# thuml/iVideoGPT

Measured on AMD Instinct MI355X. Metric: predicted frames/sec (encode+GPT rollout+decode), 64x64x16f, higher is better.
Workload: dtype bf16; 1 GPU; ivideogpt-oxe-64-act-free (BASELINE config 2): synthetic 64x64 bf16 clips, 64 trajectories per GPU, 2 context + 14 predicted frames, top-k 100 sampling, seeded random weights; global_batch=64, frames=16, resolution=64, lanes=4

## Files before the change

ivideogpt_amd/csrc/llama_ops.hip:

```cpp
#include <algorithm>
#include <cstdio>
#include <cstdlib>

#include "ops.h"
#include <atomic>
#include "switches.h"

namespace ivg {

template <typename T>
__global__ __launch_bounds__(256) void embed_kernel(const int64_t* __restrict__ ids, long id_stride, const T* __restrict__ E,
                                                    T* __restrict__ x, long x_bstride, int L, int H, int V) {
  constexpr int VEC = Traits<T>::VEC;
  const int row = blockIdx.x;
  const int b = row / L, l = row - b * L;
  long id = ids[(long)b * id_stride + l];
  id = id < 0 ? 0 : (id >= V ? V - 1 : id);
  const T* src = E + id * H;
  T* dst = x + (long)b * x_bstride + (long)l * H;
  for (int c = threadIdx.x * VEC; c < H; c += 256 * VEC) *(Chunk16*)(dst + c) = *(const Chunk16*)(src + c);
}

int launch_embed(const int64_t* ids, long id_stride, const void* E, void* x, DType dt, int B, int L, int H, int V, hipStream_t st,
                 long x_bstride) {
// ... 365 lines not shown
        }
        vf[d][pr] = bf16x8{half[0][0], half[0][1], half[0][2], half[0][3], half[1][0], half[1][1], half[1][2], half[1][3]};
      }
#pragma unroll
    for (int n = 0; n < NQ; ++n) {
      f32x4 sc[4];
      float mt = -INFINITY;
#pragma unroll
      for (int sub = 0; sub < 4; ++sub) {
        sc[sub] = f32x4{0.f, 0.f, 0.f, 0.f};
        sc[sub] = __builtin_amdgcn_mfma_f32_16x16x32_bf16(kf[sub][0], qf[n][0], sc[sub], 0, 0, 0);
        sc[sub] = __builtin_amdgcn_mfma_f32_16x16x32_bf16(kf[sub][1], qf[n][1], sc[sub], 0, 0, 0);
#pragma unroll
        for (int r = 0; r < 4; ++r) {
          const int key = k0 + sub * 16 + lg * 4 + r;
          sc[sub][r] = key <= qpos[n] ? sc[sub][r] * scale : -INFINITY;
          mt = fmaxf(mt, sc[sub][r]);
        }
      }
      mt = fmaxf(mt, __shfl_xor(mt, 16, 64));
      mt = fmaxf(mt, __shfl_xor(mt, 32, 64));
      const float mn = fmaxf(m[n], mt);
      const float ms = mn == -INFINITY ? 0.f : mn;
      const float alpha = expf(m[n] - ms);
      m[n] = mn;
      float ps = 0.f;
      bf16x8 pf[2];
#pragma unroll
      for (int sub = 0; sub < 4; ++sub)
#pragma unroll
        for (int r = 0; r < 4; ++r) {
          const float pw = expf(sc[sub][r] - ms);
          ps += pw;
          pf[sub >> 1][(sub & 1) * 4 + r] = (bf16_t)pw;
        }
      lsum[n] = lsum[n] * alpha + ps;
#pragma unroll
      for (int d = 0; d < 4; ++d) {
#pragma unroll
        for (int r = 0; r < 4; ++r) o[n][d][r] *= alpha;
#pragma unroll
        for (int pr = 0; pr < 2; ++pr) o[n][d] = __builtin_amdgcn_mfma_f32_16x16x32_bf16(vf[d][pr], pf[pr], o[n][d], 0, 0, 0);
      }
    }
  }
#pragma unroll
  for (int n = 0; n < NQ; ++n) {
    lsum[n] += __shfl_xor(lsum[n], 16, 64);
    lsum[n] += __shfl_xor(lsum[n], 32, 64);
    if (lg == 0) { sM[wave][n * 16 + lr] = m[n]; sL[wave][n * 16 + lr] = lsum[n]; }
  }
  __syncthreads();
  float* sO = (float*)sbuf;
  if (wave > 0) {
#pragma unroll
    for (int n = 0; n < NQ; ++n)
#pragma unroll
      for (int d = 0; d < 4; ++d)
#pragma unroll
        for (int r = 0; r < 4; ++r) sO[((((wave - 1) * NQ + n) * 4 + d) * 4 + r) * 64 + lane] = o[n][d][r];
  }
  __syncthreads();
  if (wave != 0) return;
#pragma unroll
  for (int n = 0; n < NQ; ++n) {
    const int qi = n * 16 + lr, t = t0 + qi;
    float M = m[n];
#pragma unroll
    for (int w = 1; w < 4; ++w) M = fmaxf(M, sM[w][qi]);
    const float s0 = expf(m[n] - M);
    float L = lsum[n] * s0;
    f32x4 acc[4];
#pragma unroll
    for (int d = 0; d < 4; ++d)
#pragma unroll
      for (int r = 0; r < 4; ++r) acc[d][r] = o[n][d][r] * s0;
#pragma unroll
    for (int w = 1; w < 4; ++w) {
      const float sw_ = expf(sM[w][qi] - M);
      L += sL[w][qi] * sw_;
#pragma unroll
      for (int d = 0; d < 4; ++d)
#pragma unroll
        for (int r = 0; r < 4; ++r) acc[d][r] += sO[((((w - 1) * NQ + n) * 4 + d) * 4 + r) * 64 + lane] * sw_;
    }
    if (t < T) {
      const float inv = 1.0f / L;
      bf16_t* orow = out + ((long)b * T + t) * H + h * HD + lg * 4;
#pragma unroll
      for (int d = 0; d < 4; ++d)
        *(bf16x4*)(orow + d * 16) = bf16x4{(bf16_t)(acc[d][0] * inv), (bf16_t)(acc[d][1] * inv), (bf16_t)(acc[d][2] * inv), (bf16_t)(acc[d][3] * inv)};
    }
  }
}

int launch_chunk_attn(const void* qkv, const void* kc, const void* vc, void* out, int B, int T, int heads, int hd, int Lmax, int pos0,
                      DType dt, hipStream_t st) {
  if (dt != BF16 || hd != 64 || B <= 0 || heads <= 0 || T < 1 || pos0 < 0 || (long)pos0 + T > Lmax) return -1;
  if (((uintptr_t)qkv & 15) || ((uintptr_t)out & 7) || ((uintptr_t)kc & 15) || ((uintptr_t)vc & 15)) return -1;
  const float scale = 1.0f / sqrtf((float)hd);
  if (T > 16)
    hipLaunchKernelGGL(chunk_attn_kernel<2>, dim3((unsigned)cdiv(T, 32), (unsigned)(B * heads)), dim3(256), 0, st, (const bf16_t*)qkv,
                       (const bf16_t*)kc, (const bf16_t*)vc, (bf16_t*)out, T, pos0, heads, Lmax, scale);
  else
    hipLaunchKernelGGL(chunk_attn_kernel<1>, dim3(1u, (unsigned)(B * heads)), dim3(256), 0, st, (const bf16_t*)qkv, (const bf16_t*)kc,
                       (const bf16_t*)vc, (bf16_t*)out, T, pos0, heads, Lmax, scale);
  return (int)hipGetLastError();
}

static std::atomic<long long> g_kv_extend_rows[2] = {{0}, {0}};
void kv_extend_note(int chunk_rows, int step_rows) { g_kv_extend_rows[0] += chunk_rows; g_kv_extend_rows[1] += step_rows; }
long long kv_extend_rows(int stepwise) { return g_kv_extend_rows[stepwise ? 1 : 0].load(); }
static std::atomic<long long> g_kv_extend_heads[2] = {{0}, {0}};
void kv_extend_heads_note(int frame_rows, int scored_rows) { g_kv_extend_heads[0] += frame_rows; g_kv_extend_heads[1] += scored_rows; }
long long kv_extend_heads_rows(int scored) { return g_kv_extend_heads[scored ? 1 : 0].load(); }

template <int HD, int KT, bool PRE = true>
__global__ __launch_bounds__(256) void xattn_kernel(const bf16_t* __restrict__ q, const bf16_t* __restrict__ Kp, const bf16_t* __restrict__ VpT,
                                                    bf16_t* __restrict__ out, int P, int kv, int C, int F, int nh, float scale) {
  constexpr int KQ = HD / 32;
  constexpr int DO = HD / 16;
  constexpr int SUB = KT / 16;
  constexpr int NPF = KT / 32;
  const int tid = threadIdx.x, wave = tid >> 6, lane = tid & 63, lr = lane & 15, lg = lane >> 4;
  const int qt = blockIdx.x;
  const int mh = blockIdx.y, m = mh / nh, h = mh - m * nh, b = m / F;
  const int qi = qt * 64 + wave * 16 + lr;
  const bf16_t* qrow = q + ((long)m * P + qi) * C + h * HD;
  bf16x8 qf[KQ];
#pragma unroll
  for (int k = 0; k < KQ; ++k) qf[k] = *(const bf16x8*)(qrow + k * 32 + lg * 8);
  const bf16_t* kb = Kp + (long)b * kv * C + h * HD;
  const bf16_t* vb = VpT + ((long)b * C + h * HD) * kv;
  f32x4 o[DO];
#pragma unroll
  for (int d = 0; d < DO; ++d) o[d] = f32x4{0.f, 0.f, 0.f, 0.f};
  float mx = -INFINITY, lsum = 0.f;
  constexpr int PK = HD + 16;
  using VT = VtTile<KT>;
  __shared__ __attribute__((aligned(16))) bf16_t sK[KT * PK];
  __shared__ __attribute__((aligned(16))) bf16_t sV[HD * VT::PITCH];
  constexpr int KC = KT * HD / 8 / 256;
  constexpr int VC = HD * KT / 8 / 256;
  constexpr int VCH = KT / 8;
  static_assert(KC >= 1 && VC >= 1, "tile too small for 256 threads");
  Chunk16 pk[KC], pvv[VC];
  auto fetch = [&](int kt) {
    const int k0 = kt * KT;
#pragma unroll
    for (int i = 0; i < KC; ++i) {
      const int c = i * 256 + tid, row = c / (HD / 8), col = (c % (HD / 8)) * 8;
      pk[i] = *(const Chunk16*)(kb + (long)(k0 + row) * C + col);
    }
#pragma unroll
    for (int i = 0; i < VC; ++i) {
      const int c = i * 256 + tid, row = c / VCH, col = (c % VCH) * 8;
      pvv[i] = *(const Chunk16*)(vb + (long)row * kv + k0 + col);
    }
  };
  const int ntiles = kv / KT;
  if constexpr (PRE) fetch(0);
  for (int kt = 0; kt < ntiles; ++kt) {
    __syncthreads();
    if constexpr (!PRE) fetch(kt);
#pragma unroll
    for (int i = 0; i < KC; ++i) { const int c = i * 256 + tid; *(Chunk16*)(sK + (c / (HD / 8)) * PK + (c % (HD / 8)) * 8) = pk[i]; }
#pragma unroll
    for (int i = 0; i < VC; ++i) { const int c = i * 256 + tid; VT::store(sV, c / VCH, c % VCH, pvv[i]); }
    __syncthreads();
    if constexpr (PRE) { if (kt + 1 < ntiles) fetch(kt + 1); }
    f32x4 sc[SUB];
    float mt = -INFINITY;
#pragma unroll
    for (int sub = 0; sub < SUB; ++sub) {
      sc[sub] = f32x4{0.f, 0.f, 0.f, 0.f};
      const bf16_t* krow = sK + (sub * 16 + lr) * PK + lg * 8;
#pragma unroll
      for (int k = 0; k < KQ; ++k) sc[sub] = __builtin_amdgcn_mfma_f32_16x16x32_bf16(*(const bf16x8*)(krow + k * 32), qf[k], sc[sub], 0, 0, 0);
#pragma unroll
      for (int r = 0; r < 4; ++r) { sc[sub][r] *= scale; mt = fmaxf(mt, sc[sub][r]); }
    }
    mt = fmaxf(mt, __shfl_xor(mt, 16, 64));
    mt = fmaxf(mt, __shfl_xor(mt, 32, 64));
    const float mn = fmaxf(mx, mt);
    const float alpha = expf(mx - mn);
    mx = mn;
    float ps = 0.f;
    bf16x8 pf[NPF];
#pragma unroll
    for (int sub = 0; sub < SUB; ++sub)
#pragma unroll
      for (int r = 0; r < 4; ++r) {
        const float pe = expf(sc[sub][r] - mn);
        ps += pe;
        pf[sub >> 1][(sub & 1) * 4 + r] = (bf16_t)pe;
      }
    lsum = lsum * alpha + ps;
#pragma unroll
    for (int d = 0; d < DO; ++d) {
#pragma unroll
      for (int r = 0; r < 4; ++r) o[d][r] *= alpha;
#pragma unroll
      for (int pr = 0; pr < NPF; ++pr)
        o[d] = __builtin_amdgcn_mfma_f32_16x16x32_bf16(VT::frag(sV, d * 16 + lr, pr * 4 + lg), pf[pr], o[d], 0, 0, 0);
    }
  }
  lsum += __shfl_xor(lsum, 16, 64);
  lsum += __shfl_xor(lsum, 32, 64);
  const float inv = 1.0f / lsum;
  bf16_t* orow = out + ((long)m * P + qi) * C + h * HD + lg * 4;
#pragma unroll
  for (int d = 0; d < DO; ++d)
    *(bf16x4*)(orow + d * 16) = bf16x4{(bf16_t)(o[d][0] * inv), (bf16_t)(o[d][1] * inv), (bf16_t)(o[d][2] * inv), (bf16_t)(o[d][3] * inv)};
}

bool xattn_covers(int P, int kv, int C, int nh, DType dt) {
  if (!sw().flash_xatt || dt != BF16 || nh <= 0 || C % nh != 0 || P % 64 != 0 || kv % 64 != 0 || (C & 7)) return false;
  const int hd = C / nh;
  return hd == 32 || hd == 64 || hd == 128 || hd == 192 || hd == 512 || hd == 768;
}

int launch_xattn(const void* q, const void* Kp, const void* VpT, void* out, int M, int F, int P, int kv, int C, int nh, DType dt, hipStream_t st) {
  if (!xattn_covers(P, kv, C, nh, dt) || M <= 0 || F <= 0 || M % F != 0) return -1;
  if (((uintptr_t)q & 15) || ((uintptr_t)Kp & 15) || ((uintptr_t)VpT & 15) || ((uintptr_t)out & 7)) return -1;
  const int hd = C / nh;
  dim3 grid((unsigned)(P / 64), (unsigned)(M * nh));
  const float scale = 1.0f / sqrtf((float)hd);
#define IVG_XATTN(HDv, KTv, PREv) hipLaunchKernelGGL((xattn_kernel<HDv, KTv, PREv>), grid, dim3(256), 0, st, (const bf16_t*)q, (const bf16_t*)Kp, (const bf16_t*)VpT, (bf16_t*)out, P, kv, C, F, nh, scale)
  if (hd == 128) IVG_XATTN(128, 64, true);
  else if (hd == 192) IVG_XATTN(192, 64, true);
  else if (hd == 64) IVG_XATTN(64, 64, true);
  else if (hd == 32) IVG_XATTN(32, 64, true);
  else if (hd == 512) IVG_XATTN(512, 32, true);
  else if (hd == 768) IVG_XATTN(768, 32, false);
  else return -1;
#undef IVG_XATTN
  return (int)hipGetLastError();
}

template <typename T> struct QPack;
template <> struct QPack<float> {
  __device__ __forceinline__ void set(const float*) {}
  __device__ __forceinline__ float dot(const float* qf, Chunk16 raw) const {
    const f32x4 kk = __builtin_bit_cast(f32x4, raw);
    float d = 0.f;
#pragma unroll
    for (int j = 0; j < 4; ++j) d = fmaf(qf[j], kk[j], d);
    return d;
  }
};
template <> struct QPack<bf16_t> {
  bf16x2 q[4];
  __device__ __forceinline__ void set(const float* qf) {
#pragma unroll
    for (int j = 0; j < 4; ++j) q[j] = bf16x2{(bf16_t)qf[2 * j], (bf16_t)qf[2 * j + 1]};
  }
  __device__ __forceinline__ float dot(const float*, Chunk16 raw) const {
    const bf16x8 kk = __builtin_bit_cast(bf16x8, raw);
    float d = 0.f;
#pragma unroll
    for (int j = 0; j < 4; ++j) d = __builtin_amdgcn_fdot2_f32_bf16(q[j], bf16x2{kk[2 * j], kk[2 * j + 1]}, d, false);
    return d;
  }
};
template <typename T> __device__ __forceinline__ float dot_chunk(const float* qf, Chunk16 raw) {
  constexpr int VEC = Traits<T>::VEC;
  float d = 0.f;
  if constexpr (sizeof(T) == 2) {
    const bf16x8 kk = __builtin_bit_cast(bf16x8, raw);
#pragma unroll
    for (int j = 0; j < VEC; ++j) d = fmaf(qf[j], (float)kk[j], d);
  } else {
    const f32x4 kk = __builtin_bit_cast(f32x4, raw);
#pragma unroll
    for (int j = 0; j < VEC; ++j) d = fmaf(qf[j], kk[j], d);
  }
  return d;
}
template <typename T> __device__ __forceinline__ void axpy_chunk(float* of, float pw, Chunk16 raw) {
  constexpr int VEC = Traits<T>::VEC;
  if constexpr (sizeof(T) == 2) {
    const bf16x8 vv = __builtin_bit_cast(bf16x8, raw);
#pragma unroll
    for (int j = 0; j < VEC; ++j) of[j] = fmaf(pw, (float)vv[j], of[j]);
  } else {
    const f32x4 vv = __builtin_bit_cast(f32x4, raw);
#pragma unroll
    for (int j = 0; j < VEC; ++j) of[j] = fmaf(pw, vv[j], of[j]);
  }
}

template <int CTRL> __device__ __forceinline__ float dpp_add(float v) {
  return v + __int_as_float(__builtin_amdgcn_update_dpp(0, __float_as_int(v), CTRL, 0xf, 0xf, false));
}
__device__ __forceinline__ float group_sum(float d, int lpk) {
  if (lpk >= 2) d = dpp_add<0xB1>(d);
  if (lpk >= 4) d = dpp_add<0x4E>(d);
  if (lpk >= 8) d = dpp_add<0x141>(d);
  if (lpk >= 16) d = dpp_add<0x140>(d);
  for (int o = 16; o < lpk; o <<= 1) d += __shfl_xor(d, o, 64);
  return d;
}

template <typename T, bool NT, int HD, bool SHARED = false>
__global__ __launch_bounds__(256) void decode_attn_kernel(const T* __restrict__ qkv, T* __restrict__ kc, T* __restrict__ vc,
                                                          T* __restrict__ out, const float* __restrict__ cosT,
                                                          const float* __restrict__ sinT, int heads, int hd_arg, int Lmax,
                                                          const StepState* __restrict__ state, unsigned long long* prof,
                                                          int sh_P = 0, int sh_G = 1, int sh_row0 = 0) {
  constexpr int VEC = Traits<T>::VEC;
  const int hd = HD > 0 ? HD : hd_arg;
  constexpr int UNR = 8;
  const unsigned long long t_start = prof ? wall_clock64() : 0ull;
  extern __shared__ __attribute__((aligned(16))) unsigned char smem[];
  const int lpk = hd / VEC;
  const int gpb = 256 / lpk;
  float* sq = (float*)smem;
  float* sk = sq + hd;
  float* sv = sk + hd;
  float* sc = sv + hd;
  float* red = sc + Lmax;
  __shared__ float sred[8];
  const int b = blockIdx.x / heads, h = blockIdx.x % heads;
  const int tid = threadIdx.x, lane = tid & 63, wv = tid >> 6;
  const int sub = tid % lpk, grp = tid / lpk;
  const int H = heads * hd, half = hd / 2;
  const float scale = rsqrtf((float)hd);
  T* kb = kc + ((long)b * heads + h) * Lmax * hd;
  T* vb = vc + ((long)b * heads + h) * Lmax * hd;
  long sh_delta = 0;
  if constexpr (SHARED) sh_delta = ((long)((b - sh_row0) / sh_G) - b) * heads * Lmax * hd * (long)sizeof(T);
  const int step = gpb * UNR;
  const unsigned lane_off = (unsigned)(sub * VEC) * (unsigned)sizeof(T);
  auto load_rows = [&](Chunk16 (&dst)[UNR], const T* base, int t0, int limit) {
    const char* bb = (const char*)base;
#pragma unroll
    for (int u = 0; u < UNR; ++u) {
      const int t = t0 + u * gpb + grp;
      const char* rb = bb;
      if constexpr (SHARED) rb = t < sh_P ? bb + sh_delta : bb;
      const Chunk16* src = (const Chunk16*)(rb + ((unsigned)(t * hd) * (unsigned)sizeof(T) + lane_off));
      dst[u] = t < limit ? ((NT && !SHARED) ? __builtin_nontemporal_load(src) : *src) : Chunk16{0u, 0u, 0u, 0u};
    }
  };
  Chunk16 cur[UNR], nxt[UNR];
  float rc = 0.f, rs = 0.f, q1 = 0.f, q2 = 0.f, k1 = 0.f, k2 = 0.f;
  T va = from_f32<T>(0.f), vb2 = from_f32<T>(0.f);
  if (tid < half) {
    const T* row = qkv + (long)b * 3 * H + h * hd;
    q1 = to_f32(row[tid]); q2 = to_f32(row[tid + half]);
    k1 = to_f32(row[H + tid]); k2 = to_f32(row[H + tid + half]);
    va = row[2 * H + tid]; vb2 = row[2 * H + tid + half];
  }
  load_rows(cur, kb, 0, Lmax);
  const int pos = state->pos;
  const int n_keys = pos + 1;
  if (tid < half) { rc = cosT[(long)pos * half + tid]; rs = sinT[(long)pos * half + tid]; }
  if (tid < half) {
    const T qa = from_f32<T>(q1 * rc - q2 * rs), qb = from_f32<T>(q2 * rc + q1 * rs);
    const T ka = from_f32<T>(k1 * rc - k2 * rs), kb2 = from_f32<T>(k2 * rc + k1 * rs);
    sq[tid] = to_f32(qa); sq[tid + half] = to_f32(qb);
    sk[tid] = to_f32(ka); sk[tid + half] = to_f32(kb2);
    sv[tid] = to_f32(va); sv[tid + half] = to_f32(vb2);
    kb[(long)pos * hd + tid] = ka; kb[(long)pos * hd + tid + half] = kb2;
    vb[(long)pos * hd + tid] = va; vb[(long)pos * hd + tid + half] = vb2;
  }
  __syncthreads();
  float qf[VEC];
#pragma unroll
  for (int j = 0; j < VEC; ++j) qf[j] = sq[sub * VEC + j];
  QPack<T> qp;
  qp.set(qf);
  auto scores = [&](Chunk16 (&rows)[UNR], int t0) {
#pragma unroll
    for (int u = 0; u < UNR; ++u) {
      const int t = t0 + u * gpb + grp;
      float d = qp.dot(qf, rows[u]);
      d = group_sum(d, lpk);
      if (t < pos && sub == 0) sc[t] = d * scale;
    }
  };
  {
    int t0 = 0;
    bool in_nxt = false;
    while (t0 < pos) {
      if (t0 + step < pos) load_rows(nxt, kb, t0 + step, pos); else load_rows(nxt, vb, 0, pos);
      scores(cur, t0);
      t0 += step;
      in_nxt = true;
      if (t0 >= pos) break;
      if (t0 + step < pos) load_rows(cur, kb, t0 + step, pos); else load_rows(cur, vb, 0, pos);
      scores(nxt, t0);
      t0 += step;
      in_nxt = false;
    }
    if (in_nxt) {
#pragma unroll
      for (int u = 0; u < UNR; ++u) cur[u] = nxt[u];
    }
  }
  if (grp == 0) {
    float d = 0.f;
#pragma unroll
    for (int j = 0; j < VEC; ++j) d = fmaf(qf[j], sk[sub * VEC + j], d);
    d = group_sum(d, lpk);
    if (sub == 0) sc[pos] = d * scale;
  }
  __syncthreads();
  float mx = -INFINITY;
  for (int t = tid; t < n_keys; t += 256) mx = fmaxf(mx, sc[t]);
  mx = wave_max(mx);
  if (lane == 0) sred[wv] = mx;
  __syncthreads();
  mx = fmaxf(fmaxf(sred[0], sred[1]), fmaxf(sred[2], sred[3]));
  float sum = 0.f;
  for (int t = tid; t < n_keys; t += 256) { const float e = expf(sc[t] - mx); sc[t] = e; sum += e; }
  sum = wave_sum(sum);
  if (lane == 0) sred[4 + wv] = sum;
  __syncthreads();
  sum = (sred[4] + sred[5]) + (sred[6] + sred[7]);
  float of[VEC];
#pragma unroll
  for (int j = 0; j < VEC; ++j) of[j] = 0.f;
  auto weighted = [&](Chunk16 (&rows)[UNR], int t0) {
#pragma unroll
    for (int u = 0; u < UNR; ++u) {
      const int t = t0 + u * gpb + grp;
      if (t < pos) axpy_chunk<T>(of, sc[t], rows[u]);
    }
  };
    for (int t0 = 0; t0 < pos; t0 += 2 * step) {
      if (t0 + step < pos) load_rows(nxt, vb, t0 + step, pos);
      weighted(cur, t0);
      if (t0 + step >= pos) break;
      if (t0 + 2 * step < pos) load_rows(cur, vb, t0 + 2 * step, pos);
      weighted(nxt, t0 + step);
    }
  if (grp == 0) {
    const float pw = sc[pos];
#pragma unroll
    for (int j = 0; j < VEC; ++j) of[j] = fmaf(pw, sv[sub * VEC + j], of[j]);
  }
#pragma unroll
  for (int j = 0; j < VEC; ++j) red[grp * hd + sub * VEC + j] = of[j];
  __syncthreads();
  if (tid < hd) {
    float a = 0.f;
    for (int g = 0; g < gpb; ++g) a += red[g * hd + tid];
    out[(long)b * H + h * hd + tid] = from_f32<T>(a / sum);
  }
  if (prof && tid == 0) {
    unsigned long long* slot = prof + (size_t)((blockIdx.x * 7 + blockIdx.y) % IVG_ATTN_PROF_SLOTS) * 2 * Lmax;
    atomicMax(slot + pos, ~t_start);
    atomicMax(slot + Lmax + pos, (unsigned long long)wall_clock64());
  }
}

bool decode_attn_covers(int hd, DType dt) {
  const int vec = dt == BF16 ? 8 : 4;
  return hd > 0 && hd <= 256 && hd % vec == 0 && 256 % (hd / vec) == 0;
}

int launch_decode_attn(const void* qkv, void* kc, void* vc, void* out, const float* cosT, const float* sinT, int B, int heads, int hd,
                       int Lmax, const StepState* state, unsigned long long* prof, DType dt, hipStream_t st, int sh_P, int sh_G, int sh_row0) {
  if (!decode_attn_covers(hd, dt)) return (int)hipErrorInvalidValue;
  const int vec = dt == BF16 ? 8 : 4;
  const int gpb = 256 / (hd / vec);
  const size_t smem = (size_t)(3 * hd + Lmax + gpb * hd) * sizeof(float);
  dim3 g(B * heads);
#define IVG_DA(T, NTv, HDv) \
  hipLaunchKernelGGL((decode_attn_kernel<T, NTv, HDv>), g, dim3(256), smem, st, (const T*)qkv, (T*)kc, (T*)vc, (T*)out, cosT, sinT, heads, hd, Lmax, state, prof, 0, 1, 0)
  if (sh_G > 1) {
    if (sh_P < 0 || sh_row0 > 0) return (int)hipErrorInvalidValue;
#define IVG_DAS(T, NTv, HDv) \
  hipLaunchKernelGGL((decode_attn_kernel<T, NTv, HDv, true>), g, dim3(256), smem, st, (const T*)qkv, (T*)kc, (T*)vc, (T*)out, cosT, sinT, heads, hd, Lmax, state, prof, sh_P, sh_G, sh_row0)
    if (dt == BF16) { if (hd == 64) IVG_DAS(bf16_t, true, 64); else IVG_DAS(bf16_t, true, 0); }
    else { if (hd == 64) IVG_DAS(float, false, 64); else IVG_DAS(float, false, 0); }
#undef IVG_DAS
    return (int)hipGetLastError();
  }
  if (dt == BF16) { if (hd == 64) IVG_DA(bf16_t, true, 64); else IVG_DA(bf16_t, true, 0); }
  else { if (hd == 64) IVG_DA(float, false, 64); else IVG_DA(float, false, 0); }
#undef IVG_DA
  return (int)hipGetLastError();
}

__device__ __forceinline__ unsigned f24_round(float x) {
  unsigned u = __float_as_uint(x);
  u += 0x7fu + ((u >> 8) & 1u);
  return u & 0xffffff00u;
}
struct Row24 { Chunk16 hi; unsigned lo0, lo1; };
__device__ __forceinline__ void row24_unpack(const Row24& r, float (&f)[8]) {
#pragma unroll
  for (int j = 0; j < 8; ++j) {
    const unsigned h = r.hi[j >> 1];
    const unsigned l = j < 4 ? r.lo0 : r.lo1;
    const unsigned sel = (j & 1) ? (0x07060000u | ((unsigned)(j & 3) << 8) | 0x0cu) : (0x05040000u | ((unsigned)(j & 3) << 8) | 0x0cu);
    f[j] = __uint_as_float(__builtin_amdgcn_perm(h, l, sel));
  }
}

template <bool SHARED>
__global__ __launch_bounds__(256) void decode_attn24_kernel(const float* __restrict__ qkv, unsigned char* __restrict__ kc, unsigned char* __restrict__ vc,
                                                            float* __restrict__ out, const float* __restrict__ cosT, const float* __restrict__ sinT,
                                                            int heads, int Lmax, const StepState* __restrict__ state, unsigned long long* prof,
                                                            int sh_P, int sh_G, int sh_row0) {
  constexpr int HD = 64, HALF = 32, LPK = 8, GPB = 32, UNR = 8;
  const unsigned long long t_start = prof ? wall_clock64() : 0ull;
  extern __shared__ __attribute__((aligned(16))) unsigned char smem[];
  float* sq = (float*)smem;
  float* sk = sq + HD;
  float* sv = sk + HD;
  float* sc = sv + HD;
  float* red = sc + Lmax;
  __shared__ float sred[8];
  const int b = blockIdx.x / heads, h = blockIdx.x % heads;
  const int tid = threadIdx.x, lane = tid & 63, wv = tid >> 6;
  const int sub = tid % LPK, grp = tid / LPK;
  const int H = heads * HD;
  const float scale = rsqrtf((float)HD);
  const long blk = (long)Lmax * (HD * 3);
  unsigned char* kb = kc + ((long)b * heads + h) * blk;
  unsigned char* vb = vc + ((long)b * heads + h) * blk;
  const unsigned lo_plane = (unsigned)Lmax * (HD * 2);
  long sh_delta = 0;
  if constexpr (SHARED) sh_delta = ((long)((b - sh_row0) / sh_G) - b) * heads * blk;
  const int step = GPB * UNR;
  auto load_rows = [&](Row24 (&dst)[UNR], const unsigned char* base, int t0, int limit) {
#pragma unroll
    for (int u = 0; u < UNR; ++u) {
      const int t = t0 + u * GPB + grp;
      const unsigned char* rb = base;
      if constexpr (SHARED) rb = t < sh_P ? base + sh_delta : base;
      const Chunk16* ph = (const Chunk16*)(rb + ((unsigned)t * (HD * 2) + (unsigned)sub * 16u));
      typedef unsigned int U2 __attribute__((ext_vector_type(2)));
      const U2* pl = (const U2*)(rb + (lo_plane + (unsigned)t * HD + (unsigned)sub * 8u));
      if (t < limit) {
        if constexpr (SHARED) { dst[u].hi = *ph; const U2 l2 = *pl; dst[u].lo0 = l2[0]; dst[u].lo1 = l2[1]; }
        else { dst[u].hi = __builtin_nontemporal_load(ph); const U2 l2 = __builtin_nontemporal_load(pl); dst[u].lo0 = l2[0]; dst[u].lo1 = l2[1]; }
      } else {
        dst[u].hi = Chunk16{0u, 0u, 0u, 0u}; dst[u].lo0 = 0u; dst[u].lo1 = 0u;
      }
    }
  };
  Row24 cur[UNR], nxt[UNR];
  float rc = 0.f, rs = 0.f, q1 = 0.f, q2 = 0.f, k1 = 0.f, k2 = 0.f, va = 0.f, vb2 = 0.f;
  if (tid < HALF) {
    const float* row = qkv + (long)b * 3 * H + h * HD;
    q1 = row[tid]; q2 = row[tid + HALF];
    k1 = row[H + tid]; k2 = row[H + tid + HALF];
    va = row[2 * H + tid]; vb2 = row[2 * H + tid + HALF];
  }
  load_rows(cur, kb, 0, Lmax);
  const int pos = state->pos;
  const int n_keys = pos + 1;
  if (tid < HALF) { rc = cosT[(long)pos * HALF + tid]; rs = sinT[(long)pos * HALF + tid]; }
  if (tid < HALF) {
    const unsigned ka = f24_round(k1 * rc - k2 * rs), kb2 = f24_round(k2 * rc + k1 * rs);
    const unsigned v1 = f24_round(va), v2 = f24_round(vb2);
    sq[tid] = q1 * rc - q2 * rs; sq[tid + HALF] = q2 * rc + q1 * rs;
    sk[tid] = __uint_as_float(ka); sk[tid + HALF] = __uint_as_float(kb2);
    sv[tid] = __uint_as_float(v1); sv[tid + HALF] = __uint_as_float(v2);
    unsigned short* kh = (unsigned short*)kb + (long)pos * HD;
    unsigned short* vh = (unsigned short*)vb + (long)pos * HD;
    unsigned char* kl = kb + lo_plane + (long)pos * HD;
    unsigned char* vl = vb + lo_plane + (long)pos * HD;
    kh[tid] = (unsigned short)(ka >> 16); kh[tid + HALF] = (unsigned short)(kb2 >> 16);
    kl[tid] = (unsigned char)(ka >> 8); kl[tid + HALF] = (unsigned char)(kb2 >> 8);
    vh[tid] = (unsigned short)(v1 >> 16); vh[tid + HALF] = (unsigned short)(v2 >> 16);
    vl[tid] = (unsigned char)(v1 >> 8); vl[tid + HALF] = (unsigned char)(v2 >> 8);
  }
  __syncthreads();
  float qf[8];
#pragma unroll
  for (int j = 0; j < 8; ++j) qf[j] = sq[sub * 8 + j];
  auto scores = [&](Row24 (&rows)[UNR], int t0) {
#pragma unroll
    for (int u = 0; u < UNR; ++u) {
      const int t = t0 + u * GPB + grp;
      float kf[8];
      row24_unpack(rows[u], kf);
      float d = 0.f;
#pragma unroll
      for (int j = 0; j < 8; ++j) d = fmaf(qf[j], kf[j], d);
      d = group_sum(d, LPK);
      if (t < pos && sub == 0) sc[t] = d * scale;
    }
  };
  {
    int t0 = 0;
    bool in_nxt = false;
    while (t0 < pos) {
      if (t0 + step < pos) load_rows(nxt, kb, t0 + step, pos); else load_rows(nxt, vb, 0, pos);
      scores(cur, t0);
      t0 += step;
      in_nxt = true;
      if (t0 >= pos) break;
      if (t0 + step < pos) load_rows(cur, kb, t0 + step, pos); else load_rows(cur, vb, 0, pos);
      scores(nxt, t0);
      t0 += step;
      in_nxt = false;
    }
    if (in_nxt) {
#pragma unroll
      for (int u = 0; u < UNR; ++u) cur[u] = nxt[u];
    }
  }
  if (grp == 0) {
    float d = 0.f;
#pragma unroll
    for (int j = 0; j < 8; ++j) d = fmaf(qf[j], sk[sub * 8 + j], d);
    d = group_sum(d, LPK);
    if (sub == 0) sc[pos] = d * scale;
  }
  __syncthreads();
  float mx = -INFINITY;
  for (int t = tid; t < n_keys; t += 256) mx = fmaxf(mx, sc[t]);
  mx = wave_max(mx);
  if (lane == 0) sred[wv] = mx;
  __syncthreads();
  mx = fmaxf(fmaxf(sred[0], sred[1]), fmaxf(sred[2], sred[3]));
  float sum = 0.f;
  for (int t = tid; t < n_keys; t += 256) { const float e = expf(sc[t] - mx); sc[t] = e; sum += e; }
  sum = wave_sum(sum);
  if (lane == 0) sred[4 + wv] = sum;
  __syncthreads();
  sum = (sred[4] + sred[5]) + (sred[6] + sred[7]);
  float of[8];
#pragma unroll
  for (int j = 0; j < 8; ++j) of[j] = 0.f;
  auto weighted = [&](Row24 (&rows)[UNR], int t0) {
#pragma unroll
    for (int u = 0; u < UNR; ++u) {
      const int t = t0 + u * GPB + grp;
      if (t < pos) {
        float vf[8];
        row24_unpack(rows[u], vf);
        const float pw = sc[t];
#pragma unroll
        for (int j = 0; j < 8; ++j) of[j] = fmaf(pw, vf[j], of[j]);
      }
    }
  };
  for (int t0 = 0; t0 < pos; t0 += 2 * step) {
    if (t0 + step < pos) load_rows(nxt, vb, t0 + step, pos);
    weighted(cur, t0);
    if (t0 + step >= pos) break;
    if (t0 + 2 * step < pos) load_rows(cur, vb, t0 + 2 * step, pos);
    weighted(nxt, t0 + step);
  }
  if (grp == 0) {
    const float pw = sc[pos];
#pragma unroll
    for (int j = 0; j < 8; ++j) of[j] = fmaf(pw, sv[sub * 8 + j], of[j]);
  }
#pragma unroll
  for (int j = 0; j < 8; ++j) red[grp * HD + sub * 8 + j] = of[j];
  __syncthreads();
  if (tid < HD) {
    float a = 0.f;
    for (int g = 0; g < GPB; ++g) a += red[g * HD + tid];
    out[(long)b * H + h * HD + tid] = a / sum;
  }
  if (prof && tid == 0) {
    unsigned long long* slot = prof + (size_t)((blockIdx.x * 7 + blockIdx.y) % IVG_ATTN_PROF_SLOTS) * 2 * Lmax;
    atomicMax(slot + pos, ~t_start);
    atomicMax(slot + Lmax + pos, (unsigned long long)wall_clock64());
  }
}

static std::atomic<long long> g_attn24_launches{0};
long long decode_attn24_launches() { return g_attn24_launches.load(); }

int launch_decode_attn24(const void* qkv, void* kc, void* vc, void* out, const float* cosT, const float* sinT, int B, int heads, int Lmax,
                         const StepState* state, unsigned long long* prof, hipStream_t st, int sh_P, int sh_G, int sh_row0) {
  g_attn24_launches.fetch_add(1, std::memory_order_relaxed);
  const size_t smem = (size_t)(3 * 64 + Lmax + 32 * 64) * sizeof(float);
  dim3 g(B * heads);
  if (sh_G > 1) {
    if (sh_P < 0 || sh_row0 > 0) return (int)hipErrorInvalidValue;
    hipLaunchKernelGGL(decode_attn24_kernel<true>, g, dim3(256), smem, st, (const float*)qkv, (unsigned char*)kc, (unsigned char*)vc, (float*)out, cosT, sinT,
                       heads, Lmax, state, prof, sh_P, sh_G, sh_row0);
  } else {
    hipLaunchKernelGGL(decode_attn24_kernel<false>, g, dim3(256), smem, st, (const float*)qkv, (unsigned char*)kc, (unsigned char*)vc, (float*)out, cosT, sinT,
                       heads, Lmax, state, prof, 0, 1, 0);
  }
  return (int)hipGetLastError();
}

__global__ __launch_bounds__(256) void kv24_pack_kernel(const float* __restrict__ k32, const float* __restrict__ v32, unsigned char* __restrict__ kc,
                                                        unsigned char* __restrict__ vc, int L, int Lmax) {
  const int bh = blockIdx.y, tid = threadIdx.x;
  const int row = blockIdx.x * 32 + (tid >> 3), sub = tid & 7;
  if (row >= L) return;
  const long blk = (long)Lmax * 192;
  const unsigned lo_plane = (unsigned)Lmax * 128u;
#pragma unroll
  for (int which = 0; which < 2; ++which) {
    const float* src = (which ? v32 : k32) + ((long)bh * Lmax + row) * 64 + sub * 8;
    unsigned char* dst = (which ? vc : kc) + (long)bh * blk;
    const f32x4 a = *(const f32x4*)src, c = *(const f32x4*)(src + 4);
    unsigned u[8];
#pragma unroll
    for (int j = 0; j < 4; ++j) { u[j] = f24_round(a[j]); u[4 + j] = f24_round(c[j]); }
    Chunk16 hi;
#pragma unroll
    for (int j = 0; j < 4; ++j) hi[j] = (u[2 * j] >> 16) | (u[2 * j + 1] & 0xffff0000u);
    uint2 lo;
    lo.x = ((u[0] >> 8) & 0xffu) | (u[1] & 0xff00u) | ((u[2] << 8) & 0xff0000u) | ((u[3] << 16) & 0xff000000u);
    lo.y = ((u[4] >> 8) & 0xffu) | (u[5] & 0xff00u) | ((u[6] << 8) & 0xff0000u) | ((u[7] << 16) & 0xff000000u);
    *(Chunk16*)(dst + (unsigned)row * 128u + (unsigned)sub * 16u) = hi;
    *(uint2*)(dst + lo_plane + (unsigned)row * 64u + (unsigned)sub * 8u) = lo;
  }
}

int launch_kv24_pack(const void* k32, const void* v32, void* kc, void* vc, int BH, int L, int Lmax, hipStream_t st) {
  if (L <= 0) return 0;
  hipLaunchKernelGGL(kv24_pack_kernel, dim3((unsigned)cdiv(L, 32), (unsigned)BH), dim3(256), 0, st, (const float*)k32, (const float*)v32, (unsigned char*)kc,
                     (unsigned char*)vc, L, Lmax);
  return (int)hipGetLastError();
}

__device__ __forceinline__ float e4m3_clamp(float x) {
  const float c = fminf(fmaxf(x, -448.f), 448.f);
  return (__float_as_uint(x) & 0x7fffffffu) > 0x7f800000u ? x : c;
}
template <bool HI> __device__ __forceinline__ int e4m3_pair(float a, float b, int old) {
  return __builtin_amdgcn_cvt_pk_fp8_f32(e4m3_clamp(a), e4m3_clamp(b), old, HI);
}
__device__ __forceinline__ void row8_unpack(const Chunk16& r, float (&f)[16]) {
#pragma unroll
  for (int w = 0; w < 4; ++w) {
    const f32x2 lo = __builtin_amdgcn_cvt_pk_f32_fp8((int)r[w], false), hi = __builtin_amdgcn_cvt_pk_f32_fp8((int)r[w], true);
    f[4 * w] = lo[0]; f[4 * w + 1] = lo[1]; f[4 * w + 2] = hi[0]; f[4 * w + 3] = hi[1];
  }
}

constexpr int KV8_LPK = 4, KV8_GPB = 256 / KV8_LPK, KV8_UNR = 8;

template <bool SHARED>
__global__ __launch_bounds__(256) void decode_attn8_kernel(const bf16_t* __restrict__ qkv, unsigned char* __restrict__ kc, unsigned char* __restrict__ vc,
                                                           bf16_t* __restrict__ out, const float* __restrict__ cosT, const float* __restrict__ sinT,
                                                           int heads, int Lmax, const StepState* __restrict__ state, unsigned long long* prof,
                                                           float k_scale, float v_scale, int sh_P, int sh_G, int sh_row0,
                                                           const float* __restrict__ ks_tab, const float* __restrict__ vs_tab) {
  constexpr int HD = 64, HALF = 32, LPK = KV8_LPK, GPB = KV8_GPB, UNR = KV8_UNR, VEC = 16;
  const unsigned long long t_start = prof ? wall_clock64() : 0ull;
  extern __shared__ __attribute__((aligned(16))) unsigned char smem[];
  float* sq = (float*)smem;
  float* sk = sq + HD;
  float* sv = sk + HD;
  float* sc = sv + HD;
  float* red = sc + Lmax;
  __shared__ float sred[8];
  const int b = blockIdx.x / heads, h = blockIdx.x % heads;
  const int tid = threadIdx.x, lane = tid & 63, wv = tid >> 6;
  const int sub = tid % LPK, grp = tid / LPK;
  const int H = heads * HD;
  if (ks_tab) { k_scale = ks_tab[h]; v_scale = vs_tab[h]; }
  const float scale = 0.125f * k_scale;
  const float inv_ks = 1.0f / k_scale, inv_vs = 1.0f / v_scale;
  const long blk = (long)Lmax * HD;
  unsigned char* kb = kc + ((long)b * heads + h) * blk;
  unsigned char* vb = vc + ((long)b * heads + h) * blk;
  long sh_delta = 0;
  if constexpr (SHARED) sh_delta = ((long)((b - sh_row0) / sh_G) - b) * heads * blk;
  const int step = GPB * UNR;
  auto load_rows = [&](Chunk16 (&dst)[UNR], const unsigned char* base, int t0, int limit) {
#pragma unroll
    for (int u = 0; u < UNR; ++u) {
      const int t = t0 + u * GPB + grp;
      const unsigned char* rb = base;
      if constexpr (SHARED) rb = t < sh_P ? base + sh_delta : base;
      const Chunk16* src = (const Chunk16*)(rb + ((unsigned)t * HD + (unsigned)sub * 16u));
      dst[u] = t < limit ? (SHARED ? *src : __builtin_nontemporal_load(src)) : Chunk16{0u, 0u, 0u, 0u};
    }
  };
  Chunk16 cur[UNR], nxt[UNR];
  float rc = 0.f, rs = 0.f, q1 = 0.f, q2 = 0.f, k1 = 0.f, k2 = 0.f, va = 0.f, vb2 = 0.f;
  if (tid < HALF) {
    const bf16_t* row = qkv + (long)b * 3 * H + h * HD;
    q1 = (float)row[tid]; q2 = (float)row[tid + HALF];
    k1 = (float)row[H + tid]; k2 = (float)row[H + tid + HALF];
// ... 1144 lines not shown
```

ivideogpt_amd/csrc/switches.cpp:

```cpp
#include "switches.h"

#include <algorithm>
#include <atomic>
#include <cstdio>
#include <cstdlib>
#include <mutex>

namespace ivg {

static int env_int(const char* name, int dflt) {
  const char* v = getenv(name);
  return (v && v[0]) ? atoi(v) : dflt;
}

static Switches read_env() {
  Switches s;
  const bool dev = env_int("IVG_DEV", 0) == 1;
  auto dv = [&](const char* name, int dflt) { return dev ? env_int(name, dflt) : dflt; };
  s.conv3x3 = dv("IVG_CONV3X3", 1) != 0;
  s.subpixel = dv("IVG_SUBPIXEL", 1) != 0;
  s.gemm256 = dv("IVG_GEMM256", 1) != 0;
  s.gemm256x3 = dv("IVG_GEMM256X3", 1) != 0;
  s.kv24 = dv("IVG_KV24", 1) != 0;
  s.dg3 = dv("IVG_DG3", 1) != 0;
  s.flash_prefill = dv("IVG_FLASH_PREFILL", 1) != 0;
  s.kv_extend_chunk = dv("IVG_KV_EXTEND_CHUNK", 1) != 0;
  s.flash_xatt = dv("IVG_FLASH_XATT", 1) != 0;
  s.gn_fuse = dv("IVG_GN_FUSE", 1) != 0;
  s.gn_apply_fuse = dv("IVG_GN_APPLY_FUSE", 1) != 0;
  s.x3 = dv("IVG_X3", 1) != 0;
  s.dg3_warm = dv("IVG_DG3_WARM", 1) != 0;
  s.warm_gate_up = dv("IVG_WARM_GATE_UP", 0) != 0;
  s.conv_cap = dv("IVG_CONV_CAP", 0) == 1;
  s.decode_w_shared = dv("IVG_DECODE_W_SHARED", 1) != 0;
  s.inflight_warm = dv("IVG_INFLIGHT_WARM", 0) != 0;
  s.dg2_mf_cap = dv("IVG_DG2_MF_CAP", 0);
  if (s.dg2_mf_cap != 1 && s.dg2_mf_cap != 2) s.dg2_mf_cap = 0;
  s.inflight_gemm256 = dv("IVG_INFLIGHT_GEMM256", 1) != 0;
  if (const char* v = dev ? getenv("IVG_INFLIGHT_KB") : nullptr) {
    int k[5] = {0, 0, 0, 0, 0};
    if (sscanf(v, "%d,%d,%d,%d,%d", &k[0], &k[1], &k[2], &k[3], &k[4]) == 5)
      for (int i = 0; i < 5; ++i) s.inflight_kb[i] = (k[i] >= 16 && k[i] <= 160) ? k[i] : 0;
  }
  s.graph = env_int("IVG_GRAPH", 0) == 1;
  s.decode_lds_kb = env_int("IVG_DECODE_LDS_KB", 160);
  if (s.decode_lds_kb < 16 || s.decode_lds_kb > 160) s.decode_lds_kb = 160;
  return s;
}

bool Switches::operator==(const Switches& o) const {
  return conv3x3 == o.conv3x3 && subpixel == o.subpixel && gemm256 == o.gemm256 && dg3 == o.dg3 && flash_prefill == o.flash_prefill &&
         flash_xatt == o.flash_xatt && gn_fuse == o.gn_fuse && gn_apply_fuse == o.gn_apply_fuse && x3 == o.x3 && gemm256x3 == o.gemm256x3 && kv24 == o.kv24 && kv_extend_chunk == o.kv_extend_chunk && graph == o.graph &&
         dg3_warm == o.dg3_warm && warm_gate_up == o.warm_gate_up && conv_cap == o.conv_cap && decode_lds_kb == o.decode_lds_kb && decode_w_shared == o.decode_w_shared &&
         inflight_warm == o.inflight_warm && dg2_mf_cap == o.dg2_mf_cap && inflight_gemm256 == o.inflight_gemm256 &&
         std::equal(inflight_kb, inflight_kb + 5, o.inflight_kb);
}

static std::atomic<const Switches*> g_cur{nullptr};
static std::atomic<unsigned> g_gen{0};
static std::mutex g_mu;

void reload_switches() {
  std::lock_guard<std::mutex> lk(g_mu);
  const Switches now = read_env();
  const Switches* cur = g_cur.load(std::memory_order_acquire);
  if (cur && *cur == now) return;
  g_cur.store(new Switches(now), std::memory_order_release);
  g_gen.fetch_add(1, std::memory_order_release);
}

const Switches& sw() {
  const Switches* p = g_cur.load(std::memory_order_acquire);
  if (!p) { reload_switches(); p = g_cur.load(std::memory_order_acquire); }
  return *p;
}

unsigned switches_generation() { return g_gen.load(std::memory_order_acquire); }

}
```

ivideogpt_amd/csrc/switches.h:

```cpp
#pragma once

namespace ivg {

struct Switches {
  int conv3x3 = 1, subpixel = 1, gemm256 = 1, dg3 = 1, flash_prefill = 1, flash_xatt = 1, gn_fuse = 1, gn_apply_fuse = 1, x3 = 1, gemm256x3 = 1, kv24 = 1, kv_extend_chunk = 1;
  int graph = 0, dg3_warm = 1, warm_gate_up = 0, conv_cap = 0, decode_lds_kb = 160, decode_w_shared = 1, inflight_warm = 0, dg2_mf_cap = 0, inflight_gemm256 = 1;
  int inflight_kb[5] = {0, 0, 0, 0, 0};
  bool operator==(const Switches& o) const;
};

const Switches& sw();
void reload_switches();
unsigned switches_generation();

}
```

Measured before the change: 5568 predicted frames/s.

## Use sliding-window buffer loads in decode attention to halve register prefetch buffers

Adds a WINDOW variant of the decode attention kernel, enabled by default for bf16 with head dim 64. Instead of double-buffering UNR rows in two register arrays, each row is reloaded right after it is consumed, using raw buffer loads whose hardware bounds check replaces the per-row branch. This frees registers and keeps loads streaming continuously. The cost is per-row load issue inside the compute loop, plus scheduling barriers that may limit overlap. The shared-prefix path needs a 32-bit offset range guard.

```diff
diff --git a/ivideogpt_amd/csrc/llama_ops.hip b/ivideogpt_amd/csrc/llama_ops.hip
--- a/ivideogpt_amd/csrc/llama_ops.hip
+++ b/ivideogpt_amd/csrc/llama_ops.hip
@@ -691,7 +691,7 @@
   return d;
 }
 
-template <typename T, bool NT, int HD, bool SHARED = false>
+template <typename T, bool NT, int HD, bool SHARED = false, bool WINDOW = false>
 __global__ __launch_bounds__(256) void decode_attn_kernel(const T* __restrict__ qkv, T* __restrict__ kc, T* __restrict__ vc,
                                                           T* __restrict__ out, const float* __restrict__ cosT,
                                                           const float* __restrict__ sinT, int heads, int hd_arg, int Lmax,
@@ -721,18 +721,25 @@
   if constexpr (SHARED) sh_delta = ((long)((b - sh_row0) / sh_G) - b) * heads * Lmax * hd * (long)sizeof(T);
   const int step = gpb * UNR;
   const unsigned lane_off = (unsigned)(sub * VEC) * (unsigned)sizeof(T);
+  auto load_row = [&](Chunk16& dst, const T* base, int t, int limit) {
+    const char* rb = (const char*)base;
+    if constexpr (SHARED) rb = t < sh_P ? rb + sh_delta : rb;
+    const Chunk16* src = (const Chunk16*)(rb + ((unsigned)(t * hd) * (unsigned)sizeof(T) + lane_off));
+    dst = t < limit ? ((NT && !SHARED) ? __builtin_nontemporal_load(src) : *src) : Chunk16{0u, 0u, 0u, 0u};
+  };
   auto load_rows = [&](Chunk16 (&dst)[UNR], const T* base, int t0, int limit) {
-    const char* bb = (const char*)base;
-#pragma unroll
-    for (int u = 0; u < UNR; ++u) {
-      const int t = t0 + u * gpb + grp;
-      const char* rb = bb;
-      if constexpr (SHARED) rb = t < sh_P ? bb + sh_delta : bb;
-      const Chunk16* src = (const Chunk16*)(rb + ((unsigned)(t * hd) * (unsigned)sizeof(T) + lane_off));
-      dst[u] = t < limit ? ((NT && !SHARED) ? __builtin_nontemporal_load(src) : *src) : Chunk16{0u, 0u, 0u, 0u};
-    }
+#pragma unroll
+    for (int u = 0; u < UNR; ++u) load_row(dst[u], base, t0 + u * gpb + grp, limit);
   };
-  Chunk16 cur[UNR], nxt[UNR];
+  const unsigned own_off = (unsigned)(-sh_delta);
+  auto win_load = [&](Chunk16& dst, const T* base, int t, int limit) {
+    const auto rsrc = __builtin_amdgcn_make_buffer_rsrc((void*)((const char*)base + sh_delta), 0,
+                                                        (int)(own_off + (unsigned)(limit * hd) * (unsigned)sizeof(T)), 0x00020000);
+    unsigned off = (unsigned)(t * hd) * (unsigned)sizeof(T) + lane_off;
+    if constexpr (SHARED) off += t < sh_P ? 0u : own_off;
+    dst = __builtin_bit_cast(Chunk16, __builtin_amdgcn_raw_buffer_load_b128(rsrc, (int)off, 0, (NT && !SHARED) ? 2 : 0));
+  };
+  Chunk16 cur[UNR], nxt[WINDOW ? 1 : UNR];
   float rc = 0.f, rs = 0.f, q1 = 0.f, q2 = 0.f, k1 = 0.f, k2 = 0.f;
   T va = from_f32<T>(0.f), vb2 = from_f32<T>(0.f);
   if (tid < half) {
@@ -741,7 +748,12 @@
     k1 = to_f32(row[H + tid]); k2 = to_f32(row[H + tid + half]);
     va = row[2 * H + tid]; vb2 = row[2 * H + tid + half];
   }
-  load_rows(cur, kb, 0, Lmax);
+  if constexpr (WINDOW) {
+#pragma unroll
+    for (int u = 0; u < UNR; ++u) win_load(cur[u], kb, u * gpb + grp, Lmax);
+  } else {
+    load_rows(cur, kb, 0, Lmax);
+  }
   const int pos = state->pos;
   const int n_keys = pos + 1;
   if (tid < half) { rc = cosT[(long)pos * half + tid]; rs = sinT[(long)pos * half + tid]; }
@@ -769,7 +781,21 @@
       if (t < pos && sub == 0) sc[t] = d * scale;
     }
   };
-  {
+  if constexpr (WINDOW) {
+    for (int t0 = 0; t0 < pos; t0 += step) {
+      const bool more = t0 + step < pos;
+      const T* nb = more ? kb : vb;
+      const int nt0 = more ? t0 + step : 0;
+#pragma unroll
+      for (int u = 0; u < UNR; ++u) {
+        const int t = t0 + u * gpb + grp;
+        float d = qp.dot(qf, cur[u]);
+        d = group_sum(d, lpk);
+        if (t < pos && sub == 0) sc[t] = d * scale;
+        win_load(cur[u], nb, nt0 + u * gpb + grp, pos);
+      }
+    }
+  } else {
     int t0 = 0;
     bool in_nxt = false;
     while (t0 < pos) {
@@ -818,6 +844,21 @@
       if (t < pos) axpy_chunk<T>(of, sc[t], rows[u]);
     }
   };
+  if constexpr (WINDOW) {
+    int t0 = 0;
+    for (; t0 + step < pos; t0 += step) {
+#pragma unroll
+      for (int u = 0; u < UNR; ++u) {
+        const int t = t0 + u * gpb + grp;
+        axpy_chunk<T>(of, sc[t], cur[u]);
+#pragma unroll
+        for (int j = 0; j < VEC; ++j) asm volatile("" : "+v"(of[j]));
+        win_load(cur[u], vb, t + step, pos);
+        __builtin_amdgcn_sched_barrier(0);
+      }
+    }
+    if (pos > 0) weighted(cur, t0);
+  } else {
     for (int t0 = 0; t0 < pos; t0 += 2 * step) {
       if (t0 + step < pos) load_rows(nxt, vb, t0 + step, pos);
       weighted(cur, t0);
@@ -825,6 +866,7 @@
       if (t0 + 2 * step < pos) load_rows(cur, vb, t0 + 2 * step, pos);
       weighted(nxt, t0 + step);
     }
+  }
   if (grp == 0) {
     const float pw = sc[pos];
 #pragma unroll
@@ -857,18 +899,24 @@
   const int gpb = 256 / (hd / vec);
   const size_t smem = (size_t)(3 * hd + Lmax + gpb * hd) * sizeof(float);
   dim3 g(B * heads);
+  const bool window = sw().decode_attn_window != 0;
 #define IVG_DA(T, NTv, HDv) \
   hipLaunchKernelGGL((decode_attn_kernel<T, NTv, HDv>), g, dim3(256), smem, st, (const T*)qkv, (T*)kc, (T*)vc, (T*)out, cosT, sinT, heads, hd, Lmax, state, prof, 0, 1, 0)
   if (sh_G > 1) {
     if (sh_P < 0 || sh_row0 > 0) return (int)hipErrorInvalidValue;
 #define IVG_DAS(T, NTv, HDv) \
   hipLaunchKernelGGL((decode_attn_kernel<T, NTv, HDv, true>), g, dim3(256), smem, st, (const T*)qkv, (T*)kc, (T*)vc, (T*)out, cosT, sinT, heads, hd, Lmax, state, prof, sh_P, sh_G, sh_row0)
-    if (dt == BF16) { if (hd == 64) IVG_DAS(bf16_t, true, 64); else IVG_DAS(bf16_t, true, 0); }
+    const bool near = sh_row0 > -sh_G && (long)B * heads * Lmax * hd * 2 < (1l << 32);
+    if (dt == BF16 && hd == 64 && window && near)
+      hipLaunchKernelGGL((decode_attn_kernel<bf16_t, true, 64, true, true>), g, dim3(256), smem, st, (const bf16_t*)qkv, (bf16_t*)kc, (bf16_t*)vc, (bf16_t*)out, cosT, sinT, heads, hd, Lmax, state, prof, sh_P, sh_G, sh_row0);
+    else if (dt == BF16) { if (hd == 64) IVG_DAS(bf16_t, true, 64); else IVG_DAS(bf16_t, true, 0); }
     else { if (hd == 64) IVG_DAS(float, false, 64); else IVG_DAS(float, false, 0); }
 #undef IVG_DAS
     return (int)hipGetLastError();
   }
-  if (dt == BF16) { if (hd == 64) IVG_DA(bf16_t, true, 64); else IVG_DA(bf16_t, true, 0); }
+  if (dt == BF16 && hd == 64 && window)
+    hipLaunchKernelGGL((decode_attn_kernel<bf16_t, true, 64, false, true>), g, dim3(256), smem, st, (const bf16_t*)qkv, (bf16_t*)kc, (bf16_t*)vc, (bf16_t*)out, cosT, sinT, heads, hd, Lmax, state, prof, 0, 1, 0);
+  else if (dt == BF16) { if (hd == 64) IVG_DA(bf16_t, true, 64); else IVG_DA(bf16_t, true, 0); }
   else { if (hd == 64) IVG_DA(float, false, 64); else IVG_DA(float, false, 0); }
 #undef IVG_DA
   return (int)hipGetLastError();
diff --git a/ivideogpt_amd/csrc/switches.cpp b/ivideogpt_amd/csrc/switches.cpp
--- a/ivideogpt_amd/csrc/switches.cpp
+++ b/ivideogpt_amd/csrc/switches.cpp
@@ -37,6 +37,7 @@
   s.dg2_mf_cap = dv("IVG_DG2_MF_CAP", 0);
   if (s.dg2_mf_cap != 1 && s.dg2_mf_cap != 2) s.dg2_mf_cap = 0;
   s.inflight_gemm256 = dv("IVG_INFLIGHT_GEMM256", 1) != 0;
+  s.decode_attn_window = dv("IVG_DECODE_ATTN_WINDOW", 1) != 0;
   if (const char* v = dev ? getenv("IVG_INFLIGHT_KB") : nullptr) {
     int k[5] = {0, 0, 0, 0, 0};
     if (sscanf(v, "%d,%d,%d,%d,%d", &k[0], &k[1], &k[2], &k[3], &k[4]) == 5)
@@ -52,7 +53,7 @@
   return conv3x3 == o.conv3x3 && subpixel == o.subpixel && gemm256 == o.gemm256 && dg3 == o.dg3 && flash_prefill == o.flash_prefill &&
          flash_xatt == o.flash_xatt && gn_fuse == o.gn_fuse && gn_apply_fuse == o.gn_apply_fuse && x3 == o.x3 && gemm256x3 == o.gemm256x3 && kv24 == o.kv24 && kv_extend_chunk == o.kv_extend_chunk && graph == o.graph &&
          dg3_warm == o.dg3_warm && warm_gate_up == o.warm_gate_up && conv_cap == o.conv_cap && decode_lds_kb == o.decode_lds_kb && decode_w_shared == o.decode_w_shared &&
-         inflight_warm == o.inflight_warm && dg2_mf_cap == o.dg2_mf_cap && inflight_gemm256 == o.inflight_gemm256 &&
+         inflight_warm == o.inflight_warm && dg2_mf_cap == o.dg2_mf_cap && inflight_gemm256 == o.inflight_gemm256 && decode_attn_window == o.decode_attn_window &&
          std::equal(inflight_kb, inflight_kb + 5, o.inflight_kb);
 }
 
diff --git a/ivideogpt_amd/csrc/switches.h b/ivideogpt_amd/csrc/switches.h
--- a/ivideogpt_amd/csrc/switches.h
+++ b/ivideogpt_amd/csrc/switches.h
@@ -4,7 +4,7 @@
 
 struct Switches {
   int conv3x3 = 1, subpixel = 1, gemm256 = 1, dg3 = 1, flash_prefill = 1, flash_xatt = 1, gn_fuse = 1, gn_apply_fuse = 1, x3 = 1, gemm256x3 = 1, kv24 = 1, kv_extend_chunk = 1;
-  int graph = 0, dg3_warm = 1, warm_gate_up = 0, conv_cap = 0, decode_lds_kb = 160, decode_w_shared = 1, inflight_warm = 0, dg2_mf_cap = 0, inflight_gemm256 = 1;
+  int graph = 0, dg3_warm = 1, warm_gate_up = 0, conv_cap = 0, decode_lds_kb = 160, decode_w_shared = 1, inflight_warm = 0, dg2_mf_cap = 0, inflight_gemm256 = 1, decode_attn_window = 1;
   int inflight_kb[5] = {0, 0, 0, 0, 0};
   bool operator==(const Switches& o) const;
 };
```

After: 5631 predicted frames/s (median of 6 runs). 1.1% higher.
